# bsxfun/pffdtd

Measured on AMD Instinct MI355X. Metric: Gvoxel-updates/s, higher is better.
Workload: dtype f32; 1 GPU; shoebox 1024^3 7-pt Cartesian fp32, Mb=11 freq-dependent walls (BASELINE.json configs[3]); Nb=12423680, Nbl=6205736, Nba=6254648, numerics=cpu-exact, parallelism=1 GPU, air_variant=0

## Files before the change

### pffdtd_amd/csrc/pf_wall.h

```cpp
#pragma once
#include <type_traits>
#include <utility>
#include "pf_kernels.h"

namespace pf {

constexpr int WALL_MAXREG = 6;
constexpr int WALL_LT = 60;
#define PF_WALL_MAXMAT 64

struct WallRegion {
   int32_t mode;
   int32_t nbase;
   int32_t kg;
   int32_t ko0, ko1;
   int32_t kb0, kb1;
   int32_t l0, l1;
   int32_t m0, m1;
   int32_t mchunk, nlt;
   int32_t nlp;
   uint32_t blk0;
   int32_t hl, lt, hm;
   int64_t pen_off;
};

template <typename Real> struct WallParams {
   const Real *A, *B;
   Real *C, *D, *E;
   int64_t plane;
   int32_t Nx, Ny, Nz, P, first, last;
   int32_t nreg;
   WallRegion reg[WALL_MAXREG];
   const uint4 *pen;
   const uint32_t *rec;
   const uint4 *blk;
   const Real *sv_in, *sg_in;
   Real *sv_out, *sg_out;
   const Real *x2, *x1;
   Real *o1, *o2, *o3;
   const Real *ssaf;
   const int8_t *mat, *Mb;
   const MatQuadT<Real> *mq;
   const Real *beta;
   Real lo2, sl2, l;
   int32_t mmax, nmat;
};

template <typename Real, int N> __device__ __forceinline__ Real wall_sel(const Real (&a)[N], int k) {
   Real r = a[0];
#pragma unroll
   for (int i = 1; i < N; i++) {
      Real t = a[i];
      asm("" : "+v"(t));
      r = (k == i) ? t : r;
   }
   return r;
}

template <typename Real> struct WallLds {
   MatQuadT<Real> mq[PF_WALL_MAXMAT * 12];
   Real beta[PF_WALL_MAXMAT];
   int32_t M[PF_WALL_MAXMAT];
};
template <typename Real> struct WallJobs {
   Real p[64 * 8];
   int32_t li[64 * 8];
   uint32_t mask[64];
};
constexpr int WALL_UROWS = 5, WALL_UROW = 12;
template <typename Real> struct WallLdsU {
   alignas(16) Real c[PF_WALL_MAXMAT][WALL_UROWS * WALL_UROW];
   Real beta[PF_WALL_MAXMAT];
   template <typename Q> __device__ __forceinline__ void put(int i, const Q &q) {
      const Real two = 2.0;
      Real *r = c[i / 12] + i % 12;
      r[0] = two * q.bDh; r[WALL_UROW] = q.bFh; r[2 * WALL_UROW] = q.b; r[3 * WALL_UROW] = q.bd; r[4 * WALL_UROW] = two * q.bFh;
   }
};
template <typename Real, int mmax, typename LDS = WallLds<Real>, int MB = mmax, bool UNI = false, bool SKIP = false>
__device__ __forceinline__ Real fd_regs(Real p, Real u2, Real sf, int32_t k, const Real (&v1)[12], const Real (&g1)[12], Real (&v1o)[12], Real (&g1o)[12],
                                        const LDS &L, Real lo2, int nb = MB) {
   if constexpr (UNI) {
      static_assert(MB >= 1 && MB <= mmax && mmax <= WALL_UROW, "uniform branch count within the state the kernel moves");
      typedef typename VecOf<Real>::type vec;
      constexpr int V = VecOf<Real>::V, NV = (MB + V - 1) / V;
      const Real two = 2.0, one = 1.0;
      const Real g = lo2 * sf * L.beta[k];
      Real cf[WALL_UROWS][NV * V];
      auto rows = [&](int32_t kk, int r0, int r1) __attribute__((always_inline)) {
         const vec *cp = (const vec *)L.c[kk];
#pragma unroll
         for (int r = r0; r < r1; r++)
#pragma unroll
            for (int v = 0; v < NV; v++) {
               const vec t = cp[r * (WALL_UROW / V) + v];
#pragma unroll
               for (int i = 0; i < V; i++) cf[r][v * V + i] = t[i];
            }
      };
      rows(k, 0, 2);
      const Real fac = two * lo2 * sf / (one + g);
      Real u = p;
      u = (u + g * u2) / (one + g);
#pragma unroll
      for (int m = 0; m < MB; m++)
         if (!SKIP || m < nb) u = u - fac * (cf[0][m] * v1[m] - cf[1][m] * g1[m]);
      const Real du = u - u2;
      int32_t k2 = k;
      asm("" : "+v"(k2) : "v"(du));
      rows(k2, 2, WALL_UROWS);
#pragma unroll
      for (int m = 0; m < MB; m++) {
         if (!SKIP || m < nb) {
            const Real v0 = cf[2][m] * du + cf[3][m] * v1[m] - cf[4][m] * g1[m];
            g1o[m] = g1[m] + (v0 + v1[m]) / two;
            v1o[m] = v0;
         } else { g1o[m] = g1[m]; v1o[m] = v1[m]; }
      }
      return u;
   } else {
      const int M = L.M[k];
      const Real two = 2.0, one = 1.0;
      const Real g = lo2 * sf * L.beta[k];
      MatQuadT<Real> q[12];
#pragma unroll
      for (int m = 0; m < 12; m++)
         if (m < mmax) q[m] = L.mq[k * 12 + m];
      const Real fac = two * lo2 * sf / (one + g);
      Real u = p;
      u = (u + g * u2) / (one + g);
#pragma unroll
      for (int m = 0; m < 12; m++) {
         if (m < mmax) {
            const Real t = u - fac * (two * q[m].bDh * v1[m] - q[m].bFh * g1[m]);
            u = (m < M) ? t : u;
         }
      }
      const Real du = u - u2;
#pragma unroll
      for (int m = 0; m < 12; m++) {
         if (m < mmax) {
            const Real v0 = q[m].b * du + q[m].bd * v1[m] - two * q[m].bFh * g1[m];
            const Real gn = g1[m] + (v0 + v1[m]) / two;
            g1o[m] = (m < M) ? gn : g1[m];
            v1o[m] = (m < M) ? v0 : v1[m];
         } else { g1o[m] = g1[m]; v1o[m] = v1[m]; }
      }
      return u;
   }
}

struct WallNodes { uint32_t x, z, w; };
struct WallProfileRow { int outer, inner; bool fd; };
constexpr int WALL_NPROF = 2;
constexpr WallProfileRow WALL_PROFILES[WALL_NPROF] = {{2, 3, true}, {2, 3, false}};
constexpr WallNodes wall_profile_words(int MODE, bool HI, int DP, int PR) {
   if (PR < 1 || PR > WALL_NPROF) return WallNodes{0u, 0u, 0u};
   const WallProfileRow r = WALL_PROFILES[PR - 1];
   const int ko = HI ? DP - 1 - r.outer : r.outer, ki = HI ? DP - 1 - r.inner : r.inner;
   const uint32_t all = 63u, no_p = all & ~(1u << (2 * MODE)), no_m = all & ~(2u << (2 * MODE));
   WallNodes n{(1u << ko) | (1u << ki), no_p | (no_m << 6), 0u};
   if (r.fd) n.w = (HI ? 1u : 2u) | ((uint32_t)ki << 8);
   return n;
}
template <int B, int E, typename F> __device__ __forceinline__ void wall_static_for(F &&f) {
   if constexpr (B < E) { f(std::integral_constant<int, B>()); wall_static_for<B + 1, E>(f); }
}

template <typename Real, int DP, int MODE, bool FAST, bool NODES, int MC, bool SG, int NS = 2, int GD = 0, bool HI = false, int PR = 0, int UB = 0, bool USK = false,
          typename LDS = WallLds<Real>>
__device__ __forceinline__ void wall_body(const WallParams<Real> &wp, const WallRegion &R, const int j, const int c, const Real a1, const Real a2,
                                          const LDS *ldsp, const uint32_t dsx, const uint32_t dsz, const uint32_t dsw, WallJobs<Real> *jobs = nullptr) {
   constexpr bool VEC = MODE == 2;
   typedef typename VecOf<Real>::type vec;
   constexpr int V = VecOf<Real>::V;
   static_assert(!VEC || DP % V == 0, "vector pencils hold whole vectors");
   const int lane = threadIdx.x;
   constexpr bool mx = MODE != 0;
   const int NL = VEC ? wp.Ny : wp.Nz;
   const int NM = mx ? wp.Nx : wp.Ny;
   const int NN = VEC ? wp.Nz : (MODE == 1 ? wp.Ny : wp.Nx);
   const bool mg_lo = mx ? (wp.first != 0) : true, mg_hi = mx ? (wp.last != 0) : true;
   const bool ng_lo = MODE == 0 ? (wp.first != 0) : true, ng_hi = MODE == 0 ? (wp.last != 0) : true;
   const int64_t sl = VEC ? (int64_t)wp.P : 1, sm = mx ? wp.plane : (int64_t)wp.P;
   const int64_t sn = VEC ? 1 : (MODE == 1 ? (int64_t)wp.P : wp.plane);
   static_assert(NS <= 2 || FAST, "three steps per pass: alike blocks only");
   const int hl = R.hl, lt = R.lt;
   const int lc = R.l0 - hl + lt * j + lane;
   int lsrc = min(max(lc, 0), NL - 1);
   if (lsrc == 0) lsrc = 2;
   else if (lsrc == NL - 1) lsrc = NL - 3;
   const bool lg_lo = lc == 0, lg_hi = lc == NL - 1;
   const bool tile_lg = !FAST && __ballot(lg_lo || lg_hi) != 0ull;
   const bool own_lane = lane >= hl && lane <= 63 - hl && lc < R.l1;
   const bool eval_lane = lane >= 1 && lane <= 62 && lc <= R.l1 + (NS == 3 ? 1 : 0);
   const int ms = R.m0 + c * R.mchunk, me = min(ms + R.mchunk, R.m1);
   if (ms >= me) return;
   const LDS &lds = *ldsp;
   constexpr int NB = UB > 0 ? UB : MC, NQ = UB > 0 ? UB : 12;
   static_assert(UB == 0 || (PR > 0 && NS == 3 && UB <= MC), "uniform branch counts: profiled three-step bodies");
   constexpr bool CG = GD > 0;
   static_assert(!CG || (FAST && NS == 3 && GD + 3 <= DP), "constant pencil geometry: alike blocks of three-step launches");
   int rkg = CG ? (HI ? DP - 1 : 0) : R.kg, rko0 = CG ? (HI ? DP - GD : 1) : R.ko0, rko1 = CG ? (HI ? DP - 1 : GD) : R.ko1;
   int rkb0 = CG ? (HI ? DP - GD - 3 : 0) : R.kb0, rkb1 = CG ? (HI ? DP : GD + 3) : R.kb1, rnbase = CG ? (HI ? NN - DP : 0) : R.nbase;
   uint32_t usx = dsx, usz = dsz, usw = dsw;
   constexpr bool PN = PR > 0;
   static_assert(!PN || (CG && NODES), "wall profiles: bodies with constant pencil geometry");
   constexpr WallNodes WN = wall_profile_words(MODE, HI, DP, PR);
   auto msrc = [&](int m) __attribute__((always_inline)) {
      m = min(max(m, 0), NM - 1);
      if (FAST) return m;
      if (m == 0 && mg_lo) return 2;
      if (m == NM - 1 && mg_hi) return NM - 3;
      return m;
   };
   const int64_t lbase = (int64_t)lsrc * sl + (int64_t)rnbase * sn;
   const int ql = (lc == 1 || lc == NL - 2) ? 1 : 0;
   const bool tile_ql = !FAST && __ballot(ql != 0) != 0ull;

   auto load_pencil = [&](const Real *G, int m, Real(&b)[DP]) __attribute__((always_inline)) {
      const Real *pl = G + (int64_t)msrc(m) * sm + lbase;
      if constexpr (VEC) {
#pragma unroll
         for (int v = 0; v < DP / V; v++) {
            const vec t = *(const vec *)(pl + v * V);
#pragma unroll
            for (int i = 0; i < V; i++) b[v * V + i] = t[i];
         }
      } else {
#pragma unroll
         for (int k = 0; k < DP; k++) b[k] = pl[(int64_t)min(max(k, rkb0), rkb1 - 1) * sn];
      }
   };
   auto mirror = [&](Real(&b)[DP]) __attribute__((always_inline)) {
#pragma unroll
      for (int k = DP - 1; k >= 0; k--) {
         const Real src = (k == 0) ? b[2] : b[k >= 2 ? k - 2 : 0];
         b[k] = (k == rkg) ? src : b[k];
      }
   };
   auto load_ent = [&](int m) __attribute__((always_inline)) {
      const uint4 *e = wp.pen + (R.pen_off + (int64_t)(min(m, R.m1 + R.hm - 1) - (R.m0 - R.hm)) * R.nlp + (lt * j + lane));
      if (FAST && (!NODES || (PN && (WN.w & 31u) == 0u))) return make_uint4(0u, 0u, 0u, 0u);
      if (FAST) return make_uint4(0u, 0u, 0u, e->w);
      return *e;
   };
   auto mask_ent = [&](uint4 e, int m) __attribute__((always_inline)) {
      if (!eval_lane || m > R.m1 + (NS == 3 ? 1 : 0)) { e.x = 0u; e.w = 0u; }
      return e;
   };
   auto store_pencil = [&](Real *G, int m, const Real(&v)[DP]) __attribute__((always_inline)) {
      if (!own_lane) return;
      Real *pl = G + (int64_t)m * sm + (int64_t)lc * sl + (int64_t)rnbase * sn;
      if constexpr (VEC) {
#pragma unroll
         for (int q = 0; q < DP / V; q++) {
            if ((q + 1) * V > rko0 && q * V < rko1) {
               vec t;
#pragma unroll
               for (int i = 0; i < V; i++) t[i] = (rkg > 0 && q * V + i > rkg) ? Real(0) : v[q * V + i];
               *(vec *)(pl + q * V) = t;
            }
         }
      } else {
#pragma unroll
         for (int k = 0; k < DP; k++)
            if (k >= rko0 && k < rko1) pl[(int64_t)k * sn] = v[k];
      }
   };
   auto fd_fetch = [&](const uint4 E, Real(&v)[12], Real(&g)[12], Real &sf, Real &u2, Real &x1v, int32_t &k) __attribute__((always_inline)) {
      if (NODES && (E.w & 31u) != 0u) {
         const int32_t li = (int32_t)(E.w >> 8);
#pragma unroll
         for (int m = 0; m < 12; m++)
            if (m < NB) { v[m] = wp.sv_in[st_idx(m, li)]; g[m] = wp.sg_in[st_idx(m, li)]; }
         sf = wp.ssaf[li];
         k = wp.mat[li];
         u2 = wp.x2[li];
         x1v = wp.x1[li];
      }
   };
   auto air = [&](Real cc, Real old, Real np_, Real nm, Real mp, Real mm, Real lp, Real lm) __attribute__((always_inline)) {
      if (MODE == 2) return upd7<SG>(a1, a2, cc, old, mp, mm, lp, lm, np_, nm);
      if (MODE == 1) return upd7<SG>(a1, a2, cc, old, mp, mm, np_, nm, lp, lm);
      return upd7<SG>(a1, a2, cc, old, np_, nm, mp, mm, lp, lm);
   };
   auto rigid = [&](uint32_t adj, Real cc, Real old, Real np_, Real nm, Real mp, Real mm, Real lp, Real lm) __attribute__((always_inline)) {
      Real nb[6];
      if (MODE == 2) { nb[0] = mp; nb[1] = mm; nb[2] = lp; nb[3] = lm; nb[4] = np_; nb[5] = nm; }
      else if (MODE == 1) { nb[0] = mp; nb[1] = mm; nb[2] = np_; nb[3] = nm; nb[4] = lp; nb[5] = lm; }
      else { nb[0] = np_; nb[1] = nm; nb[2] = mp; nb[3] = mm; nb[4] = lp; nb[5] = lm; }
      return upd_rigid<SG, 6>(a2, wp.sl2, adj, cc, old, nb);
   };

   auto update = [&](auto stage, int m, const Real(&Prv)[DP], const Real(&Cur)[DP], const Real(&Nxt)[DP], const Real(&Old)[DP], const uint4 E,
                     Real(&Out)[DP], bool own_m, const Real(&Fv)[12], const Real(&Fg)[12], Real(&Fvo)[12], Real(&Fgo)[12], Real Fsf, Real Fu2,
                     int32_t Fk, Real &nval, bool &st) __attribute__((always_inline)) {
      constexpr int STAGE = decltype(stage)::value;
      if constexpr (FAST) {
         st = false;
         if constexpr (PN) {
            constexpr uint32_t sx = WN.x, sw5 = WN.w & 31u;
            constexpr int sk0 = (int)(WN.w >> 8);
            Real pfd = Real(0);
            wall_static_for<1, DP - 1>([&](auto kc) __attribute__((always_inline)) {
               constexpr int k = decltype(kc)::value;
               const Real cc = Cur[k];
               const Real lm = lane_from_lower<true>(cc), lp = lane_from_upper<true>(cc);
               Real p;
               if constexpr (((sx >> k) & 1u) != 0u) {
                  constexpr uint32_t jn = k == 0 ? 0u : (uint32_t)__builtin_popcount(sx & ((1u << k) - 1u));
                  p = rigid((WN.z >> (6 * jn)) & 63u, cc, Old[k], Cur[k + 1], Cur[k - 1], Nxt[k], Prv[k], lp, lm);
                  if constexpr (sw5 != 0u && k == sk0) pfd = p;
               } else {
                  p = air(cc, Old[k], Cur[k + 1], Cur[k - 1], Nxt[k], Prv[k], lp, lm);
                  if constexpr (k == 1) { if (__builtin_expect(!HI && ng_lo, 0)) p = abc_loss<SG>(p, Old[k], wp.l); }
               }
               Out[k] = p;
            });
            static_assert(((sx >> 1) & 1u) == 0u && ((sx >> (DP - 2)) & 1u) == 0u, "wall profiles: no node on the ABC cell");
            if (HI && ng_hi) Out[DP - 2] = abc_loss<SG>(Out[DP - 2], Old[DP - 2], wp.l);
            if constexpr (sw5 != 0u) {
               const bool owner = own_m && own_lane && sk0 >= rko0 && sk0 < rko1;
               if (eval_lane && (STAGE < NS || STAGE == 1 || owner)) {
                  if constexpr (UB > 0) pfd = fd_regs<Real, MC, LDS, UB, true, USK>(pfd, Fu2, Fsf, Fk, Fv, Fg, Fvo, Fgo, lds, wp.lo2, USK ? wp.mmax : UB);
                  else pfd = fd_regs<Real, MC>(pfd, Fu2, Fsf, Fk, Fv, Fg, Fvo, Fgo, lds, wp.lo2);
                  st = owner;
                  nval = pfd;
               }
               Out[sk0] = pfd;
            }
            mirror(Out);
            return;
         }
         const uint32_t sx = NODES ? usx : 0u, sw5 = NODES ? (usw & 31u) : 0u, sk0 = usw >> 8;
         Real pfd = Real(0);
#pragma unroll
         for (int k = 1; k < DP - 1; k++) {
            const Real cc = Cur[k];
            const Real lm = lane_from_lower<true>(cc), lp = lane_from_upper<true>(cc);
            Real p = air(cc, Old[k], Cur[k + 1], Cur[k - 1], Nxt[k], Prv[k], lp, lm);
            if (k == 1) {
               const int nk = rnbase + k;
               const bool abc1 = CG ? (!HI && ng_lo) : ((ng_lo && nk == 1) || (ng_hi && nk == NN - 2));
               if (__builtin_expect(abc1, 0)) p = abc_loss<SG>(p, Old[k], wp.l);
            }
            if (NODES && __builtin_expect(((sx >> k) & 1u) != 0u, 0)) {
               const uint32_t jn = __popc(sx & ((1u << k) - 1u));
               p = rigid((usz >> (6 * jn)) & 63u, cc, Old[k], Cur[k + 1], Cur[k - 1], Nxt[k], Prv[k], lp, lm);
               if ((uint32_t)k == sk0) pfd = p;
            }
            Out[k] = p;
         }
         if constexpr (CG) {
            if (HI && ng_hi && !(NODES && ((sx >> (DP - 2)) & 1u))) Out[DP - 2] = abc_loss<SG>(Out[DP - 2], Old[DP - 2], wp.l);
         } else {
            const int kh = NN - 2 - rnbase;
            if (ng_hi && kh >= 2 && kh <= DP - 2 && !(NODES && ((sx >> kh) & 1u))) {
               const Real t = abc_loss<SG>(wall_sel<Real, DP>(Out, kh), wall_sel<Real, DP>(Old, kh), wp.l);
#pragma unroll
               for (int k = 2; k < DP - 1; k++) Out[k] = (k == kh) ? t : Out[k];
            }
         }
         if (NODES && sw5 != 0u) {
            const bool owner = own_m && own_lane && (int)sk0 >= rko0 && (int)sk0 < rko1;
            if (eval_lane && (STAGE < NS || STAGE == 1 || owner)) {
               if constexpr (UB == 0) pfd = fd_regs<Real, MC>(pfd, Fu2, Fsf, Fk, Fv, Fg, Fvo, Fgo, lds, wp.lo2);
               st = owner;
               nval = pfd;
            }
#pragma unroll
            for (int k = 1; k < DP - 1; k++) Out[k] = ((uint32_t)k == sk0) ? pfd : Out[k];
         }
         mirror(Out);
         return;
      }
      const int qm = FAST ? 0 : (mx ? (((wp.first && m == 1) || (wp.last && m == wp.Nx - 2)) ? 1 : 0) : ((m == 1 || m == wp.Ny - 2) ? 1 : 0));
      st = false;
      const uint32_t sx = !NODES ? 0u : FAST ? usx : __builtin_amdgcn_readlane(E.x, 1), sz = FAST ? usz : __builtin_amdgcn_readlane(E.z, 1);
      const uint32_t sw5 = !NODES ? 0u : FAST ? (usw & 31u) : (__builtin_amdgcn_readlane(E.w, 1) & 31u), sk0 = FAST ? (usw >> 8) : (__builtin_amdgcn_readlane(E.y, 1) >> 27);
      bool alike = true;
      if (!FAST) {
         const bool differs = eval_lane && (E.x != sx || E.z != sz || (E.w & 31u) != sw5 || (E.y >> 27) != sk0);
         alike = __ballot(differs) == 0ull && __popc(sx) <= 5 && __popc(sw5) <= 1;
      }
      Real pfd = Real(0);
#pragma unroll
      for (int k = 1; k < DP - 1; k++) {
         const Real cc = Cur[k];
         const Real lm = lane_from_lower<true>(cc), lp = lane_from_upper<true>(cc);
         Real p = Real(0);
         const int nk = rnbase + k;
         const bool node_all = alike && ((sx >> k) & 1u);
         if (!node_all) {
            p = air(cc, Old[k], Cur[k + 1], Cur[k - 1], Nxt[k], Prv[k], lp, lm);
            const int qnm = (((ng_lo && nk == 1) || (ng_hi && nk == NN - 2)) ? 1 : 0) + qm;
            if (qnm > 0 || tile_ql) {
               const int Q = qnm + (FAST ? 0 : ql);
               if (Q > 0) p = abc_loss<SG>(p, Old[k], wp.l * (Real)Q);
            }
         }
         if (node_all) {
            const uint32_t jn = __popc(sx & ((1u << k) - 1u));
            p = rigid((sz >> (6 * jn)) & 63u, cc, Old[k], Cur[k + 1], Cur[k - 1], Nxt[k], Prv[k], lp, lm);
            if (sw5 != 0u && (uint32_t)k == sk0) pfd = p;
         }
         Out[k] = p;
      }
      if (alike) {
         if (sw5 != 0u) {
            const bool owner = own_m && own_lane && (int)sk0 >= rko0 && (int)sk0 < rko1;
            if (eval_lane && (STAGE == 1 || owner)) {
               if constexpr (UB == 0) pfd = fd_regs<Real, MC>(pfd, Fu2, Fsf, Fk, Fv, Fg, Fvo, Fgo, lds, wp.lo2);
               st = owner;
               nval = pfd;
            }
#pragma unroll
            for (int k = 1; k < DP - 1; k++)
               if ((uint32_t)k == sk0) Out[k] = pfd;
         }
      } else if (!FAST) {
         uint32_t ub = 0;
#pragma unroll
         for (int k = 1; k < DP - 1; k++)
            if (__ballot((E.x >> k) & 1u) != 0ull) ub |= 1u << k;
         const int k0 = (int)(E.y >> 27);
         uint32_t jm = 0u;
         constexpr bool BATCH = DP <= 8;
         while (ub) {
            const int k = __ffs(ub) - 1;
            ub &= ub - 1u;
            const bool has = ((E.x >> k) & 1u) != 0u;
            const int jn = __popc(E.x & ((1u << k) - 1u));
            const bool inl = jn < 5;
            const bool lossy_inl = inl && ((E.w >> jn) & 1u) != 0u;
            const bool prim = has && lossy_inl && k == k0;
            const bool need_rec = has && (!inl || (lossy_inl && !prim));
            uint32_t rec = 0u;
            if (__ballot(need_rec) != 0ull) {
               if (need_rec) rec = wp.rec[(E.y & 0x7ffffffu) + (uint32_t)jn];
            }
            const uint32_t adj = inl ? ((E.z >> (6 * jn)) & 63u) : (rec & 63u);
            const Real cc = wall_sel<Real, DP>(Cur, k), nm = wall_sel<Real, DP>(Cur, k - 1), np_ = wall_sel<Real, DP>(Cur, k + 1);
            const Real mp = wall_sel<Real, DP>(Nxt, k), mm = wall_sel<Real, DP>(Prv, k), old = wall_sel<Real, DP>(Old, k);
            const Real lm = lane_from_lower<true>(cc), lp = lane_from_upper<true>(cc);
            Real p = rigid(adj, cc, old, np_, nm, mp, mm, lp, lm);
            const bool owner = own_m && own_lane && k >= rko0 && k < rko1;
            if (prim && (STAGE == 1 || owner)) {
               if constexpr (UB == 0) p = fd_regs<Real, MC>(p, Fu2, Fsf, Fk, Fv, Fg, Fvo, Fgo, lds, wp.lo2);
               st = owner;
               nval = p;
            }
            const bool fds = has && !prim && (inl ? lossy_inl : (rec & 64u) != 0u) && (STAGE == 1 || owner);
            if (BATCH) {
               if (fds) {
                  jobs->p[lane * 8 + k] = p;
                  jobs->li[lane * 8 + k] = (int32_t)(rec >> 8) | (owner ? (1 << 30) : 0);
                  jm |= 1u << k;
               }
            } else if (__ballot(fds) != 0ull) {
               if (fds) {
                  const int32_t li = (int32_t)(rec >> 8);
                  const Real u2 = STAGE == 1 ? wp.x2[li] : wp.x1[li];
                  p = fd_core<Real>(p, u2, li, STAGE == 1 ? wp.sv_in : wp.sv_out, STAGE == 1 ? wp.sg_in : wp.sg_out, wp.sv_out, wp.sg_out, owner, wp.ssaf,
                                    wp.mat, wp.Mb, wp.mq, wp.beta, wp.lo2, wp.mmax);
                  if (owner) (STAGE == 1 ? wp.o1 : wp.o2)[li] = p;
               }
            }
#pragma unroll
            for (int i = 1; i < DP - 1; i++) Out[i] = (has && k == i) ? p : Out[i];
         }
         if (BATCH && __ballot(jm != 0u) != 0ull) {
            jobs->mask[lane] = jm;
            __syncthreads();
            for (int t = 0; t < 8; t++) {
               const int slot = t * 64 + lane, src = slot >> 3, kk = slot & 7;
               const bool valid = ((jobs->mask[src] >> kk) & 1u) != 0u;
               if (__ballot(valid) != 0ull) {
                  if (valid) {
                     const int32_t w = jobs->li[slot], li = w & 0x3fffffff;
                     const bool own = (w >> 30) != 0;
                     const Real u2 = STAGE == 1 ? wp.x2[li] : wp.x1[li];
                     const Real r = fd_core<Real>(jobs->p[slot], u2, li, STAGE == 1 ? wp.sv_in : wp.sv_out, STAGE == 1 ? wp.sg_in : wp.sg_out, wp.sv_out, wp.sg_out, own,
                                                  wp.ssaf, wp.mat, wp.Mb, wp.mq, wp.beta, wp.lo2, wp.mmax);
                     if (own) (STAGE == 1 ? wp.o1 : wp.o2)[li] = r;
                     jobs->p[slot] = r;
                  }
               }
            }
            __syncthreads();
#pragma unroll
            for (int i = 1; i < DP - 1; i++)
               if ((jm >> i) & 1u) Out[i] = jobs->p[lane * 8 + i];
            __syncthreads();
         }
      }
      mirror(Out);
      if (STAGE == 1 && tile_lg) {
#pragma unroll
         for (int k = 0; k < DP; k++) {
            const Real t = Out[k];
            const Real up = __shfl(t, lane + 2, 64), dn = __shfl(t, lane - 2, 64);
            Out[k] = lg_lo ? up : (lg_hi ? dn : t);
         }
      }
   };

   Real Bm[DP], Bc[DP], Bn[DP], Bq[DP], Ac[DP], Aq[DP], Vm[DP], Vc[DP], Vn[DP], W[DP];
   Real Xm[NS == 3 ? DP : 1], Xc[NS == 3 ? DP : 1], Y[NS == 3 ? DP : 1];
   Real F1v[12], F1g[12], Fqv[12], Fqg[12], F2v[12], F2g[12];
   Real F3v[NS == 3 ? 12 : 1], F3g[NS == 3 ? 12 : 1];
   Real F1sf = 0, F1u2 = 0, F1x1 = 0, Fqsf = 0, Fqu2 = 0, Fqx1 = 0, F2sf = 0, F2u2 = 0, F3sf = 0, F3u2 = 0, F2n1 = 0;
   int32_t F1k = 0, Fqk = 0, F2k = 0, F3k = 0;
#pragma unroll
   for (int q = 0; q < 12; q++) { F1v[q] = F1g[q] = Fqv[q] = Fqg[q] = F2v[q] = F2g[q] = Real(0); if (NS == 3) F3v[q] = F3g[q] = Real(0); }
   const int mf = NS == 1 ? ms : ms - (NS - 1), ml = NS == 1 ? me - 1 : me + (NS - 2);
   uint4 Epp = make_uint4(0u, 0u, 0u, 0u), Ep = make_uint4(0u, 0u, 0u, 0u), Ec = mask_ent(load_ent(mf), mf), En = mask_ent(load_ent(mf + 1), mf + 1), Eq;
   load_pencil(wp.B, mf - 1, Bm);
   load_pencil(wp.B, mf, Bc);
   load_pencil(wp.B, mf + 1, Bn);
   load_pencil(wp.A, mf, Ac);
   mirror(Bm); mirror(Bc); mirror(Bn);
   fd_fetch(Ec, F1v, F1g, F1sf, F1u2, F1x1, F1k);
#pragma unroll
   for (int k = 0; k < DP; k++) { Vm[k] = Real(0); Vc[k] = Real(0); Vn[k] = Real(0); W[k] = Real(0); }
   if constexpr (NS == 3) {
#pragma unroll
      for (int k = 0; k < DP; k++) { Xm[k] = Real(0); Xc[k] = Real(0); Y[k] = Real(0); }
   }
   Eq = load_ent(mf + 2);
   load_pencil(wp.B, mf + 2, Bq);
   load_pencil(wp.A, mf + 1, Aq);
   fd_fetch(En, Fqv, Fqg, Fqsf, Fqu2, Fqx1, Fqk);
   for (int m = mf; m <= ml; m++) {
      usx = dsx; usz = dsz; usw = dsw;
      if constexpr (PN) {}
      else if constexpr (CG) asm volatile("" : "+s"(usx), "+s"(usz), "+s"(usw));
      else {
         rkg = R.kg; rko0 = R.ko0; rko1 = R.ko1; rkb0 = R.kb0; rkb1 = R.kb1; rnbase = R.nbase;
         asm volatile("" : "+s"(rkg), "+s"(rko0), "+s"(rko1), "+s"(rkb0), "+s"(rkb1), "+s"(rnbase), "+s"(usx), "+s"(usz), "+s"(usw));
      }
      const bool own_m = m >= ms && m < me;
      Real nv1 = Real(0), nv2 = Real(0), nv3 = Real(0);
      bool st1 = false, st2 = false, st3 = false;
      update(std::integral_constant<int, 1>(), m, Bm, Bc, Bn, Ac, Ec, Vn, own_m, F1v, F1g, F1v, F1g, F1sf, F1u2, F1k, nv1, st1);
      if constexpr (PN) {}
      else if constexpr (CG) asm volatile("" : "+s"(usx), "+s"(usz), "+s"(usw));
      else asm volatile("" : "+s"(rkg), "+s"(rko0), "+s"(rko1), "+s"(rnbase), "+s"(usx), "+s"(usz), "+s"(usw));
      const bool do2 = NS >= 2 && m - 1 >= ms - (NS - 2);
      const bool own_m2 = m - 1 >= ms && m - 1 < me;
      if (do2) {
         if (!mx && !FAST) {
            const bool sub_hi = m == NM - 1 && mg_hi, sub_lo = m - 2 == 0 && mg_lo;
            Real Pv[DP], Nv[DP];
#pragma unroll
            for (int k = 0; k < DP; k++) { Pv[k] = sub_lo ? Vn[k] : Vm[k]; Nv[k] = sub_hi ? Vm[k] : Vn[k]; }
            update(std::integral_constant<int, 2>(), m - 1, Pv, Vc, Nv, Bm, Ep, W, true, F2v, F2g, F2v, F2g, F2sf, F2u2, F2k, nv2, st2);
         } else update(std::integral_constant<int, 2>(), m - 1, Vm, Vc, Vn, Bm, Ep, W, own_m2, F2v, F2g, F2v, F2g, F2sf, F2u2, F2k, nv2, st2);
      }
      const bool do3 = NS == 3 && m - 2 >= ms;
      if constexpr (NS == 3) {
         if constexpr (PN) {}
         else if constexpr (CG) asm volatile("" : "+s"(usx), "+s"(usz), "+s"(usw));
         else asm volatile("" : "+s"(rkg), "+s"(rko0), "+s"(rko1), "+s"(rnbase), "+s"(usx), "+s"(usz), "+s"(usw));
         if (do3) update(std::integral_constant<int, 3>(), m - 2, Xm, Xc, W, Vm, Epp, Y, true, F3v, F3g, F3v, F3g, F3sf, F3u2, F3k, nv3, st3);
      }
      const int32_t li1 = (int32_t)(Ec.w >> 8), li2 = (int32_t)(Ep.w >> 8), li3 = (int32_t)(Epp.w >> 8);
#pragma unroll
      for (int k = 0; k < DP; k++) { Vm[k] = Vc[k]; Vc[k] = Vn[k]; Bm[k] = Bc[k]; Bc[k] = Bn[k]; Bn[k] = Bq[k]; Ac[k] = Aq[k]; }
#pragma unroll
      for (int k = 0; k < DP; k++) { asm volatile("" : "+v"(Bn[k])); asm volatile("" : "+v"(Ac[k])); }
#pragma unroll
      for (int q = 0; q < NQ; q++) { asm volatile("" : "+v"(Fqv[q])); asm volatile("" : "+v"(Fqg[q])); }
      asm volatile("" : "+v"(Fqsf), "+v"(Fqu2), "+v"(Fqx1), "+v"(Fqk), "+v"(Eq.x), "+v"(Eq.y), "+v"(Eq.z), "+v"(Eq.w) : : "memory");
      mirror(Bn);
      if constexpr (UB > 0) { if (own_m && wp.C) store_pencil(wp.C, m, Vc); }
      else if (own_m) store_pencil(wp.C, m, Vc);
      if (do2 && own_m2) store_pencil(wp.D, m - 1, W);
      if constexpr (NS == 3) { if (do3) store_pencil(wp.E, m - 2, Y); }
      if (st1) wp.o1[li1] = nv1;
      if (NS == 1 && st1) {
#pragma unroll
         for (int q = 0; q < 12; q++)
            if (q < MC) { wp.sv_out[st_idx(q, li1)] = F1v[q]; wp.sg_out[st_idx(q, li1)] = F1g[q]; }
      }
      if (st2) {
         wp.o2[li2] = nv2;
         if (NS == 2) {
#pragma unroll
            for (int q = 0; q < 12; q++)
               if (q < MC) { wp.sv_out[st_idx(q, li2)] = F2v[q]; wp.sg_out[st_idx(q, li2)] = F2g[q]; }
         }
      }
      if constexpr (NS == 3) {
         if (st3) {
            wp.o3[li3] = nv3;
#pragma unroll
            for (int q = 0; q < 12; q++)
               if (q < NB) { wp.sv_out[st_idx(q, li3)] = F3v[q]; wp.sg_out[st_idx(q, li3)] = F3g[q]; }
         }
      }
      asm volatile("" : : : "memory");
      if constexpr (NS == 3) {
#pragma unroll
         for (int k = 0; k < DP; k++) { Xm[k] = Xc[k]; Xc[k] = W[k]; }
#pragma unroll
         for (int q = 0; q < NQ; q++) { F3v[q] = F2v[q]; F3g[q] = F2g[q]; }
         F3sf = F2sf; F3k = F2k; F3u2 = F2n1;
         F2n1 = nv1;
      }
#pragma unroll
      for (int q = 0; q < NQ; q++) { F2v[q] = F1v[q]; F2g[q] = F1g[q]; F1v[q] = Fqv[q]; F1g[q] = Fqg[q]; }
      F2sf = F1sf; F2u2 = F1x1; F2k = F1k;
      F1sf = Fqsf; F1u2 = Fqu2; F1x1 = Fqx1; F1k = Fqk;
      Epp = Ep; Ep = Ec; Ec = En; En = mask_ent(Eq, m + 2);
      if (m + 1 <= ml) {
         Eq = load_ent(m + 3);
         if (m + 1 < ml) {
            load_pencil(wp.B, m + 3, Bq);
            load_pencil(wp.A, m + 2, Aq);
            fd_fetch(En, Fqv, Fqg, Fqsf, Fqu2, Fqx1, Fqk);
         }
      }
   }
}

template <typename Real, int DP, bool VEC, bool FAST, bool NODES = true, int MC = 12, bool SG = false, int NS = 2, int GD = 0, int PR = 0, int UB = 0, bool USK = false>
__global__ __launch_bounds__(64) __attribute__((amdgpu_waves_per_eu((FAST && !VEC && NS != 3 && sizeof(Real) == 4) ? 2 : 1))) void k_wall2(WallParams<Real> wp, Real a1, Real a2) {
   static_assert(FAST || NODES, "generic blocks have everything");
   const uint4 bd = wp.blk[blockIdx.x];
   const WallRegion R = wp.reg[bd.x & 7u];
   const int j = (int)((bd.x >> 3) & 0x1fffu), c = (int)(bd.x >> 16);
   typedef typename std::conditional<(UB > 0), WallLdsU<Real>, WallLds<Real>>::type LDS;
   __shared__ LDS lds;
   __shared__ typename std::conditional<FAST, int, WallJobs<Real>>::type jobs_mem;
   WallJobs<Real> *jobs = nullptr;
   if constexpr (!FAST) {
      jobs = &jobs_mem;
      jobs->mask[threadIdx.x] = 0u;
   }
   if constexpr (UB > 0) {
      for (int i = threadIdx.x; i < wp.nmat * 12; i += 64) lds.put(i, wp.mq[i]);
      for (int i = threadIdx.x; i < wp.nmat; i += 64) lds.beta[i] = wp.beta[i];
      __syncthreads();
   } else if (NODES) {
      for (int i = threadIdx.x; i < wp.nmat * 12; i += 64) lds.mq[i] = wp.mq[i];
      for (int i = threadIdx.x; i < wp.nmat; i += 64) { lds.beta[i] = wp.beta[i]; lds.M[i] = wp.Mb[i]; }
      __syncthreads();
   }
   static_assert(PR == 0 || GD > 0, "wall profiles: with constant pencil geometry");
   if constexpr (GD > 0) {
      const bool hi = R.kg != 0;
      if constexpr (VEC) { if (hi) wall_body<Real, DP, 2, FAST, NODES, MC, SG, NS, GD, true, PR, UB, USK, LDS>(wp, R, j, c, a1, a2, &lds, bd.y, bd.z, bd.w, jobs);
                           else wall_body<Real, DP, 2, FAST, NODES, MC, SG, NS, GD, false, PR, UB, USK, LDS>(wp, R, j, c, a1, a2, &lds, bd.y, bd.z, bd.w, jobs); }
      else if (R.mode == 1) { if (hi) wall_body<Real, DP, 1, FAST, NODES, MC, SG, NS, GD, true, PR, UB, USK, LDS>(wp, R, j, c, a1, a2, &lds, bd.y, bd.z, bd.w, jobs);
                              else wall_body<Real, DP, 1, FAST, NODES, MC, SG, NS, GD, false, PR, UB, USK, LDS>(wp, R, j, c, a1, a2, &lds, bd.y, bd.z, bd.w, jobs); }
      else { if (hi) wall_body<Real, DP, 0, FAST, NODES, MC, SG, NS, GD, true, PR, UB, USK, LDS>(wp, R, j, c, a1, a2, &lds, bd.y, bd.z, bd.w, jobs);
             else wall_body<Real, DP, 0, FAST, NODES, MC, SG, NS, GD, false, PR, UB, USK, LDS>(wp, R, j, c, a1, a2, &lds, bd.y, bd.z, bd.w, jobs); }
   } else if constexpr (VEC) wall_body<Real, DP, 2, FAST, NODES, MC, SG, NS>(wp, R, j, c, a1, a2, &lds, bd.y, bd.z, bd.w, jobs);
   else if (R.mode == 1) wall_body<Real, DP, 1, FAST, NODES, MC, SG, NS>(wp, R, j, c, a1, a2, &lds, bd.y, bd.z, bd.w, jobs);
   else wall_body<Real, DP, 0, FAST, NODES, MC, SG, NS>(wp, R, j, c, a1, a2, &lds, bd.y, bd.z, bd.w, jobs);
}

struct WallKernel { int dp = 0; bool vec = false, fast = false, nodes = false; int mc = 0, ns = 0, gd = 0, pr = 0, ub = 0; bool usk = false; };
constexpr int WALL_MC[2] = {4, 12};
constexpr int wall_mc(int mb_max) { return mb_max <= WALL_MC[0] ? WALL_MC[0] : WALL_MC[1]; }
constexpr int WALL_DP[4] = {8, 12, 16, 20}, WALL_DP3 = 10;
template <int N> struct WallKernelTable { WallKernel k[N]; int n = 0; static constexpr int cap = N; constexpr void add(const WallKernel &w) { k[n++] = w; } };
template <bool F64> constexpr auto wall_kernels() {
   WallKernelTable<F64 ? 28 : 60> t{};
   for (int gi = 0; gi < (F64 ? 3 : 4); gi++) for (int mc : WALL_MC) {
      const int dp = WALL_DP[gi], d3 = gi == 0 ? WALL_DP3 : dp, gd = gi == 0 ? 6 : 16; const bool vec = gi != 0, lo = mc == WALL_MC[0];
      for (int ns = 1; ns <= 2; ns++) {
         t.add({dp, vec, true, true, mc, ns}); t.add({dp, vec, false, true, mc, ns}); if (vec && !lo) t.add({dp, vec, true, false, mc, ns});
      }
      if (F64 || (gi != 0 && gi != 3)) continue;
      if (gi == 0) t.add({d3, vec, true, true, mc, 2});
      t.add({d3, vec, true, true, mc, 3}); t.add({d3, vec, true, true, mc, 3, gd}); t.add({d3, vec, true, true, mc, 3, gd, 1});
      if (lo) { t.add({d3, vec, true, true, mc, 3, gd, 2}); t.add({d3, vec, true, true, mc, 3, gd, 1, mc, true}); }
      else { t.add({d3, vec, true, true, mc, 3, gd, 1, 11}); t.add({d3, vec, true, true, mc, 3, gd, 1, 12}); }
   }
   return t;
}
template <bool F64> inline constexpr auto WALL_KERNELS = wall_kernels<F64>();
template <bool F64> constexpr const WallKernel *wall_choose(int gi, int q, int ns, int mb_max, bool ns3, bool ns3z, int geo, int prof, int uni) {
   constexpr auto &T = WALL_KERNELS<F64>;
   if (ns == 3 && !(gi == 0 ? ns3 : gi == 3 && ns3z)) return nullptr;
   const int dp = gi == 0 && ns3 ? WALL_DP3 : WALL_DP[gi];
   const WallKernel *best = nullptr; int most = -1;
   for (const WallKernel &r : T.k) {
      if (r.dp != dp || r.ns != ns || r.fast != (q != 1) || r.nodes != (q != 2)) continue;
      const bool bound = r.nodes && r.ub == 0 && !(r.pr > 0 && !WALL_PROFILES[r.pr - 1].fd);
      const int facts = (r.gd > 0) + (r.pr > 0) + (r.ub > 0);
      if ((r.gd == 0 || r.gd == geo) && (r.pr == 0 || r.pr == prof) && (r.ub == 0 || (uni > 0 && (r.usk ? uni <= r.ub : uni == r.ub))) && (!bound || r.mc == wall_mc(mb_max)) && facts > most) { best = &r; most = facts; }
   }
   return best;
}
template <bool F64> constexpr bool wall_choices_match_table() {
   constexpr auto &T = WALL_KERNELS<F64>;
   bool hit[T.cap] = {}, gv[WALL_DP[3] + 2] = {true}, mv[WALL_MC[1] + 2] = {true};
   for (const WallKernel &r : T.k) { gv[r.gd] = gv[r.gd + 1] = mv[r.mc] = mv[r.mc + 1] = mv[r.ub] = mv[r.ub + 1] = true; }
   for (int gi = 0; gi < 4; gi++) for (int q = 0; q < 3; q++) for (int ns = 1; ns <= 3; ns++) for (int t = 0; t < 3; t++) {
      const bool t3 = gi == 0 ? t > 0 : (gi == 3 && t > 1 && ns == 3);
      const bool none = t3 ? (F64 || q != 0 || ns == 1) : (ns == 3 || (gi == 0 && q == 2) || (F64 && gi == 3));
      for (int mb = 0; mb <= WALL_MC[1]; mb++) for (int uni = 0; mv[mb] && uni <= (ns == 3 ? mb : 0); uni += mb ? mb : 1)
         for (int geo = 0; geo <= (ns == 3 ? WALL_DP[3] : 0); geo++) for (int prof = 0; gv[geo] && prof <= (ns == 3 ? WALL_NPROF : 0); prof++) {
            const WallKernel *k = wall_choose<F64>(gi, q, ns, mb, t > 0, t > 1, geo, prof, uni);
            if (none != !k) return false; else if (k) hit[k - T.k] = true;
         }
   }
   for (bool h : hit) if (!h) return false;
   return true;
}
static_assert(wall_choices_match_table<false>(), "k_wall2, fp32: the chooser and the table of instantiations disagree");
static_assert(wall_choices_match_table<true>(), "k_wall2, fp64: the chooser and the table of instantiations disagree");
template <typename Real, bool SG, int... I> void wall_launch(const WallKernel *k, dim3 grid, hipStream_t st, const WallParams<Real> &wp, Real a1, Real a2, std::integer_sequence<int, I...>) {
   constexpr auto &T = WALL_KERNELS<sizeof(Real) == 8>;
   (void)((k == &T.k[I] && (k_wall2<Real, T.k[I].dp, T.k[I].vec, T.k[I].fast, T.k[I].nodes, T.k[I].mc, SG, T.k[I].ns, T.k[I].gd, T.k[I].pr, T.k[I].ub, T.k[I].usk><<<grid, dim3(64), 0, st>>>(wp, a1, a2), true)) || ...);
}
}
```

Measured before the change: 845.8 Gvoxel-updates/s.

## Pack wall branch state into float pairs and reuse per-node coefficients across stages

For the uniform-branch wall kernels, the branch state (v, g) now lives in two-wide float vectors so the per-branch updates can map to packed-math instructions. The g and fac coefficients computed in stage one are carried along the pipeline and reused in later stages instead of being recomputed (which involved a division). The branch updates are now guarded by a wavefront ballot, and the second coefficient-row load is split to shorten live ranges. The unused NS<3 state stores are compiled out for this path. Risks include register pressure from the extra carried scalars and the compiler failing to emit packed ops.

```diff
diff --git a/pffdtd_amd/csrc/pf_wall.h b/pffdtd_amd/csrc/pf_wall.h
--- a/pffdtd_amd/csrc/pf_wall.h
+++ b/pffdtd_amd/csrc/pf_wall.h
@@ -68,6 +68,24 @@
    uint32_t mask[64];
 };
 constexpr int WALL_UROWS = 5, WALL_UROW = 12;
+template <typename Real> struct WallPair { typedef Real type __attribute__((ext_vector_type(2))); };
+template <typename Real, int N> struct WallPairs {
+   static constexpr int NP = N / 2;
+   typename WallPair<Real>::type p[NP > 0 ? NP : 1];
+   Real s;
+   __device__ __forceinline__ Real get(int m) const { return m < 2 * NP ? p[m / 2][m % 2] : s; }
+   __device__ __forceinline__ void set(int m, Real x) { if (m < 2 * NP) p[m / 2][m % 2] = x; else s = x; }
+   __device__ __forceinline__ void zero() {
+#pragma unroll
+      for (int j = 0; j < (NP > 0 ? NP : 1); j++) p[j] = Real(0);
+      s = Real(0);
+   }
+   __device__ __forceinline__ void touch() {
+#pragma unroll
+      for (int j = 0; j < NP; j++) asm volatile("" : "+v"(p[j]));
+      if (N % 2) asm volatile("" : "+v"(s));
+   }
+};
 template <typename Real> struct WallLdsU {
    alignas(16) Real c[PF_WALL_MAXMAT][WALL_UROWS * WALL_UROW];
    Real beta[PF_WALL_MAXMAT];
@@ -77,45 +95,75 @@
       r[0] = two * q.bDh; r[WALL_UROW] = q.bFh; r[2 * WALL_UROW] = q.b; r[3 * WALL_UROW] = q.bd; r[4 * WALL_UROW] = two * q.bFh;
    }
 };
-template <typename Real, int mmax, typename LDS = WallLds<Real>, int MB = mmax, bool UNI = false, bool SKIP = false>
-__device__ __forceinline__ Real fd_regs(Real p, Real u2, Real sf, int32_t k, const Real (&v1)[12], const Real (&g1)[12], Real (&v1o)[12], Real (&g1o)[12],
-                                        const LDS &L, Real lo2, int nb = MB) {
+template <typename Real, int mmax, typename LDS = WallLds<Real>, int MB = mmax, bool UNI = false, bool SKIP = false, bool HAVE = false, typename ST = Real[12]>
+__device__ __forceinline__ Real fd_regs(Real p, Real u2, Real sf, int32_t k, const ST &v1, const ST &g1, ST &v1o, ST &g1o, const LDS &L, Real lo2, int nb = MB, Real *cg = nullptr, Real *cfac = nullptr) {
    if constexpr (UNI) {
       static_assert(MB >= 1 && MB <= mmax && mmax <= WALL_UROW, "uniform branch count within the state the kernel moves");
       typedef typename VecOf<Real>::type vec;
-      constexpr int V = VecOf<Real>::V, NV = (MB + V - 1) / V;
+      typedef typename WallPair<Real>::type pair;
+      constexpr int V = VecOf<Real>::V, NV = (MB + V - 1) / V, NP = MB / 2;
+      constexpr bool TAIL = MB % 2 != 0;
+      static_assert(V % 2 == 0 && std::is_same<ST, WallPairs<Real, MB>>::value, "the state arrives as pairs of branches");
       const Real two = 2.0, one = 1.0;
-      const Real g = lo2 * sf * L.beta[k];
-      Real cf[WALL_UROWS][NV * V];
-      auto rows = [&](int32_t kk, int r0, int r1) __attribute__((always_inline)) {
+      Real g, fac;
+      if constexpr (HAVE) { g = *cg; fac = *cfac; }
+      else g = lo2 * sf * L.beta[k];
+      pair cf[WALL_UROWS][NV * V / 2];
+      auto rows = [&](int32_t kk, int r0, int r1, int va, int vb) __attribute__((always_inline)) {
          const vec *cp = (const vec *)L.c[kk];
 #pragma unroll
          for (int r = r0; r < r1; r++)
 #pragma unroll
-            for (int v = 0; v < NV; v++) {
+            for (int v = va; v < vb; v++) {
                const vec t = cp[r * (WALL_UROW / V) + v];
 #pragma unroll
-               for (int i = 0; i < V; i++) cf[r][v * V + i] = t[i];
+               for (int i = 0; i < V / 2; i++) cf[r][v * (V / 2) + i] = pair{t[2 * i], t[2 * i + 1]};
             }
       };
-      rows(k, 0, 2);
-      const Real fac = two * lo2 * sf / (one + g);
+      rows(k, 0, 2, 0, NV);
+      if constexpr (!HAVE) {
+         fac = two * lo2 * sf / (one + g);
+         if (cg) { *cg = g; *cfac = fac; }
+      }
       Real u = p;
       u = (u + g * u2) / (one + g);
+      pair t[NP > 0 ? NP : 1];
+      Real ts = Real(0);
+#pragma unroll
+      for (int j = 0; j < NP; j++)
+         if (!SKIP || 2 * j < nb) t[j] = fac * (cf[0][j] * v1.p[j] - cf[1][j] * g1.p[j]);
+      if constexpr (TAIL) { if (!SKIP || MB - 1 < nb) ts = fac * (cf[0][NP].x * v1.s - cf[1][NP].x * g1.s); }
 #pragma unroll
       for (int m = 0; m < MB; m++)
-         if (!SKIP || m < nb) u = u - fac * (cf[0][m] * v1[m] - cf[1][m] * g1[m]);
+         if (!SKIP || m < nb) u = u - (m < 2 * NP ? t[m / 2][m % 2] : ts);
       const Real du = u - u2;
       int32_t k2 = k;
       asm("" : "+v"(k2) : "v"(du));
-      rows(k2, 2, WALL_UROWS);
-#pragma unroll
-      for (int m = 0; m < MB; m++) {
-         if (!SKIP || m < nb) {
-            const Real v0 = cf[2][m] * du + cf[3][m] * v1[m] - cf[4][m] * g1[m];
-            g1o[m] = g1[m] + (v0 + v1[m]) / two;
-            v1o[m] = v0;
-         } else { g1o[m] = g1[m]; v1o[m] = v1[m]; }
+      rows(k2, 2, WALL_UROWS, 0, NV < 2 ? NV : 2);
+#pragma unroll
+      for (int j = 0; j < NP; j++) {
+         if (NV > 2 && j * 2 == V) {
+            int32_t k3 = k;
+            asm("" : "+v"(k3) : "v"(g1o.p[V / 2 - 1]));
+            rows(k3, 2, WALL_UROWS, 2, NV);
+         }
+         if (!SKIP || 2 * j < nb) {
+            const pair v0 = cf[2][j] * du + cf[3][j] * v1.p[j] - cf[4][j] * g1.p[j];
+            const pair gn = g1.p[j] + (v0 + v1.p[j]) / two;
+            if (!SKIP || 2 * j + 1 < nb) { g1o.p[j] = gn; v1o.p[j] = v0; }
+            else {
+               pair go = g1.p[j], vo = v1.p[j];
+               go.x = gn.x; vo.x = v0.x;
+               g1o.p[j] = go; v1o.p[j] = vo;
+            }
+         } else { g1o.p[j] = g1.p[j]; v1o.p[j] = v1.p[j]; }
+      }
+      if constexpr (TAIL) {
+         if (!SKIP || MB - 1 < nb) {
+            const Real v0 = cf[2][NP].x * du + cf[3][NP].x * v1.s - cf[4][NP].x * g1.s;
+            g1o.s = g1.s + (v0 + v1.s) / two;
+            v1o.s = v0;
+         } else { g1o.s = g1.s; v1o.s = v1.s; }
       }
       return u;
    } else {
@@ -198,6 +246,7 @@
    if (ms >= me) return;
    const LDS &lds = *ldsp;
    constexpr int NB = UB > 0 ? UB : MC, NQ = UB > 0 ? UB : 12;
+   Real Fcg[3] = {}, Fcf[3] = {};
    static_assert(UB == 0 || (PR > 0 && NS == 3 && UB <= MC), "uniform branch counts: profiled three-step bodies");
    constexpr bool CG = GD > 0;
    static_assert(!CG || (FAST && NS == 3 && GD + 3 <= DP), "constant pencil geometry: alike blocks of three-step launches");
@@ -268,12 +317,15 @@
             if (k >= rko0 && k < rko1) pl[(int64_t)k * sn] = v[k];
       }
    };
-   auto fd_fetch = [&](const uint4 E, Real(&v)[12], Real(&g)[12], Real &sf, Real &u2, Real &x1v, int32_t &k) __attribute__((always_inline)) {
+   auto fd_fetch = [&](const uint4 E, auto &v, auto &g, Real &sf, Real &u2, Real &x1v, int32_t &k) __attribute__((always_inline)) {
       if (NODES && (E.w & 31u) != 0u) {
          const int32_t li = (int32_t)(E.w >> 8);
 #pragma unroll
          for (int m = 0; m < 12; m++)
-            if (m < NB) { v[m] = wp.sv_in[st_idx(m, li)]; g[m] = wp.sg_in[st_idx(m, li)]; }
+            if (m < NB) {
+               if constexpr (UB > 0) { v.set(m, wp.sv_in[st_idx(m, li)]); g.set(m, wp.sg_in[st_idx(m, li)]); }
+               else { v[m] = wp.sv_in[st_idx(m, li)]; g[m] = wp.sg_in[st_idx(m, li)]; }
+            }
          sf = wp.ssaf[li];
          k = wp.mat[li];
          u2 = wp.x2[li];
@@ -294,7 +346,7 @@
    };
 
    auto update = [&](auto stage, int m, const Real(&Prv)[DP], const Real(&Cur)[DP], const Real(&Nxt)[DP], const Real(&Old)[DP], const uint4 E,
-                     Real(&Out)[DP], bool own_m, const Real(&Fv)[12], const Real(&Fg)[12], Real(&Fvo)[12], Real(&Fgo)[12], Real Fsf, Real Fu2,
+                     Real(&Out)[DP], bool own_m, const auto &Fv, const auto &Fg, auto &Fvo, auto &Fgo, Real Fsf, Real Fu2,
                      int32_t Fk, Real &nval, bool &st) __attribute__((always_inline)) {
       constexpr int STAGE = decltype(stage)::value;
       if constexpr (FAST) {
@@ -322,9 +374,15 @@
             if (HI && ng_hi) Out[DP - 2] = abc_loss<SG>(Out[DP - 2], Old[DP - 2], wp.l);
             if constexpr (sw5 != 0u) {
                const bool owner = own_m && own_lane && sk0 >= rko0 && sk0 < rko1;
-               if (eval_lane && (STAGE < NS || STAGE == 1 || owner)) {
-                  if constexpr (UB > 0) pfd = fd_regs<Real, MC, LDS, UB, true, USK>(pfd, Fu2, Fsf, Fk, Fv, Fg, Fvo, Fgo, lds, wp.lo2, USK ? wp.mmax : UB);
-                  else pfd = fd_regs<Real, MC>(pfd, Fu2, Fsf, Fk, Fv, Fg, Fvo, Fgo, lds, wp.lo2);
+               if constexpr (UB > 0) {
+                  const bool need = eval_lane && (STAGE < NS || STAGE == 1 || owner);
+                  if (__ballot(need) != 0ull) {
+                     pfd = fd_regs<Real, MC, LDS, UB, true, USK, (STAGE > 1)>(pfd, Fu2, Fsf, Fk, Fv, Fg, Fvo, Fgo, lds, wp.lo2, USK ? wp.mmax : UB, &Fcg[STAGE - 1], &Fcf[STAGE - 1]);
+                     st = owner;
+                     nval = pfd;
+                  }
+               } else if (eval_lane && (STAGE < NS || STAGE == 1 || owner)) {
+                  pfd = fd_regs<Real, MC>(pfd, Fu2, Fsf, Fk, Fv, Fg, Fvo, Fgo, lds, wp.lo2);
                   st = owner;
                   nval = pfd;
                }
@@ -508,12 +566,18 @@
 
    Real Bm[DP], Bc[DP], Bn[DP], Bq[DP], Ac[DP], Aq[DP], Vm[DP], Vc[DP], Vn[DP], W[DP];
    Real Xm[NS == 3 ? DP : 1], Xc[NS == 3 ? DP : 1], Y[NS == 3 ? DP : 1];
-   Real F1v[12], F1g[12], Fqv[12], Fqg[12], F2v[12], F2g[12];
-   Real F3v[NS == 3 ? 12 : 1], F3g[NS == 3 ? 12 : 1];
+   typedef typename std::conditional<(UB > 0), WallPairs<Real, NQ>, Real[12]>::type FState;
+   typedef typename std::conditional<(UB > 0), WallPairs<Real, NQ>, Real[NS == 3 ? 12 : 1]>::type FState3;
+   FState F1v, F1g, Fqv, Fqg, F2v, F2g;
+   FState3 F3v, F3g;
    Real F1sf = 0, F1u2 = 0, F1x1 = 0, Fqsf = 0, Fqu2 = 0, Fqx1 = 0, F2sf = 0, F2u2 = 0, F3sf = 0, F3u2 = 0, F2n1 = 0;
    int32_t F1k = 0, Fqk = 0, F2k = 0, F3k = 0;
-#pragma unroll
-   for (int q = 0; q < 12; q++) { F1v[q] = F1g[q] = Fqv[q] = Fqg[q] = F2v[q] = F2g[q] = Real(0); if (NS == 3) F3v[q] = F3g[q] = Real(0); }
+   if constexpr (UB > 0) {
+      F1v.zero(); F1g.zero(); Fqv.zero(); Fqg.zero(); F2v.zero(); F2g.zero(); F3v.zero(); F3g.zero();
+   } else {
+#pragma unroll
+      for (int q = 0; q < 12; q++) { F1v[q] = F1g[q] = Fqv[q] = Fqg[q] = F2v[q] = F2g[q] = Real(0); if (NS == 3) F3v[q] = F3g[q] = Real(0); }
+   }
    const int mf = NS == 1 ? ms : ms - (NS - 1), ml = NS == 1 ? me - 1 : me + (NS - 2);
    uint4 Epp = make_uint4(0u, 0u, 0u, 0u), Ep = make_uint4(0u, 0u, 0u, 0u), Ec = mask_ent(load_ent(mf), mf), En = mask_ent(load_ent(mf + 1), mf + 1), Eq;
    load_pencil(wp.B, mf - 1, Bm);
@@ -570,8 +634,11 @@
       for (int k = 0; k < DP; k++) { Vm[k] = Vc[k]; Vc[k] = Vn[k]; Bm[k] = Bc[k]; Bc[k] = Bn[k]; Bn[k] = Bq[k]; Ac[k] = Aq[k]; }
 #pragma unroll
       for (int k = 0; k < DP; k++) { asm volatile("" : "+v"(Bn[k])); asm volatile("" : "+v"(Ac[k])); }
-#pragma unroll
-      for (int q = 0; q < NQ; q++) { asm volatile("" : "+v"(Fqv[q])); asm volatile("" : "+v"(Fqg[q])); }
+      if constexpr (UB > 0) { Fqv.touch(); Fqg.touch(); }
+      else {
+#pragma unroll
+         for (int q = 0; q < NQ; q++) { asm volatile("" : "+v"(Fqv[q])); asm volatile("" : "+v"(Fqg[q])); }
+      }
       asm volatile("" : "+v"(Fqsf), "+v"(Fqu2), "+v"(Fqx1), "+v"(Fqk), "+v"(Eq.x), "+v"(Eq.y), "+v"(Eq.z), "+v"(Eq.w) : : "memory");
       mirror(Bn);
       if constexpr (UB > 0) { if (own_m && wp.C) store_pencil(wp.C, m, Vc); }
@@ -579,17 +646,21 @@
       if (do2 && own_m2) store_pencil(wp.D, m - 1, W);
       if constexpr (NS == 3) { if (do3) store_pencil(wp.E, m - 2, Y); }
       if (st1) wp.o1[li1] = nv1;
-      if (NS == 1 && st1) {
-#pragma unroll
-         for (int q = 0; q < 12; q++)
-            if (q < MC) { wp.sv_out[st_idx(q, li1)] = F1v[q]; wp.sg_out[st_idx(q, li1)] = F1g[q]; }
+      if constexpr (UB == 0) {
+         if (NS == 1 && st1) {
+#pragma unroll
+            for (int q = 0; q < 12; q++)
+               if (q < MC) { wp.sv_out[st_idx(q, li1)] = F1v[q]; wp.sg_out[st_idx(q, li1)] = F1g[q]; }
+         }
       }
       if (st2) {
          wp.o2[li2] = nv2;
-         if (NS == 2) {
-#pragma unroll
-            for (int q = 0; q < 12; q++)
-               if (q < MC) { wp.sv_out[st_idx(q, li2)] = F2v[q]; wp.sg_out[st_idx(q, li2)] = F2g[q]; }
+         if constexpr (UB == 0) {
+            if (NS == 2) {
+#pragma unroll
+               for (int q = 0; q < 12; q++)
+                  if (q < MC) { wp.sv_out[st_idx(q, li2)] = F2v[q]; wp.sg_out[st_idx(q, li2)] = F2g[q]; }
+            }
          }
       }
       if constexpr (NS == 3) {
@@ -597,20 +668,31 @@
             wp.o3[li3] = nv3;
 #pragma unroll
             for (int q = 0; q < 12; q++)
-               if (q < NB) { wp.sv_out[st_idx(q, li3)] = F3v[q]; wp.sg_out[st_idx(q, li3)] = F3g[q]; }
+               if (q < NB) {
+                  if constexpr (UB > 0) { wp.sv_out[st_idx(q, li3)] = F3v.get(q); wp.sg_out[st_idx(q, li3)] = F3g.get(q); }
+                  else { wp.sv_out[st_idx(q, li3)] = F3v[q]; wp.sg_out[st_idx(q, li3)] = F3g[q]; }
+               }
          }
       }
       asm volatile("" : : : "memory");
       if constexpr (NS == 3) {
 #pragma unroll
          for (int k = 0; k < DP; k++) { Xm[k] = Xc[k]; Xc[k] = W[k]; }
-#pragma unroll
-         for (int q = 0; q < NQ; q++) { F3v[q] = F2v[q]; F3g[q] = F2g[q]; }
+         if constexpr (UB > 0) { F3v = F2v; F3g = F2g; }
+         else {
+#pragma unroll
+            for (int q = 0; q < NQ; q++) { F3v[q] = F2v[q]; F3g[q] = F2g[q]; }
+         }
+         if constexpr (UB > 0) { Fcg[2] = Fcg[1]; Fcf[2] = Fcf[1]; }
          F3sf = F2sf; F3k = F2k; F3u2 = F2n1;
          F2n1 = nv1;
       }
-#pragma unroll
-      for (int q = 0; q < NQ; q++) { F2v[q] = F1v[q]; F2g[q] = F1g[q]; F1v[q] = Fqv[q]; F1g[q] = Fqg[q]; }
+      if constexpr (UB > 0) { F2v = F1v; F2g = F1g; F1v = Fqv; F1g = Fqg; }
+      else {
+#pragma unroll
+         for (int q = 0; q < NQ; q++) { F2v[q] = F1v[q]; F2g[q] = F1g[q]; F1v[q] = Fqv[q]; F1g[q] = Fqg[q]; }
+      }
+      if constexpr (UB > 0) { Fcg[1] = Fcg[0]; Fcf[1] = Fcf[0]; }
       F2sf = F1sf; F2u2 = F1x1; F2k = F1k;
       F1sf = Fqsf; F1u2 = Fqu2; F1x1 = Fqx1; F1k = Fqk;
       Epp = Ep; Ep = Ec; Ec = En; En = mask_ent(Eq, m + 2);
```

Result: no change. 845.1 Gvoxel-updates/s (-0.1%).
